# demorest/dspsr

Measured on AMD Instinct MI355X. Metric: Msamples/s dedispersed+folded, higher is better.
Workload: dtype f32

## Files before the change

dspsr_amd/csrc/fb_common.h:

```cpp
#pragma once
#include <math.h>
#include <stdlib.h>

#include <vector>

#include "engine_internal.h"
#include "fold_internal.h"
#include "stamps.h"

namespace dspsr_amd {

struct FbGeom {
  int logM, logR, logT1, logT2, logT3;
  int logX3;
  int four_pass;
  int xblocked;
  uint32_t xblock;
  uint32_t kblock;
  uint64_t xstride;
  int logMf, logMa, logMb, logTm, logTt;
  int real_input, npol;
  uint32_t nsub;
  int logFb2, logFa2;
  uint32_t C, nfilt_pos, nkeep;
  const float2* tw_lo;
  const float2* tw_lo_m;
};

struct FbIn {
  int kind;
  const void* base;
  uint64_t pol_stride;
  uint64_t part_step;
  uint32_t nchan, ichan;
  float scale;
  uint32_t batch;
  uint64_t chan_stride_c;
};

struct FbOut {
  int kind;
  float* base;
  uint64_t chan_stride, pol_stride, part_step;
  int state;
  uint32_t ndim, chan0;
  uint32_t nbin;
  uint64_t prof_span4;
  uint32_t prof_planes;
  uint64_t plane_stride;
  float* part;
  uint32_t nchan_prof;
  uint32_t nseg;
  dspsr_amd_fold* fold;
  const uint32_t* pstart;
  uint32_t nparts_plan;
  uint32_t plan_cap;
  const Interval* piv;
  const uint32_t* blk_first;
  const uint32_t* bin_start;
  uint32_t ts_sf;
  uint32_t ts_magic;
  uint32_t ts_phase0;
  uint32_t ts_G;
  float* ts_carry;
};

struct TsPart { uint32_t phi, ng, rlast, ofirst; };
DEV TsPart ts_part(const FbOut& out, const uint32_t part_in_call, const uint32_t nkeep)
{
  const uint32_t s = out.ts_phase0 + part_in_call * nkeep;
  TsPart p;
  p.ofirst = s / out.ts_sf;
  p.phi = s - p.ofirst * out.ts_sf;
  const uint32_t e = p.phi + nkeep;
  p.ng = (e + out.ts_sf - 1) / out.ts_sf;
  p.rlast = e - (p.ng - 1) * out.ts_sf;
  return p;
}
DEV float sqld(const cf a) { return __fadd_rn(__fmul_rn(a.x, a.x), __fmul_rn(a.y, a.y)); }
DEV void ts_stage(float* __restrict__ stg, const FbOut& out, const TsPart& tp, const uint32_t slo, const uint32_t t, const cf a, const cf b)
{
  const uint32_t tr = t + tp.phi, gq = out.ts_sf == 1 ? tr : __umulhi(tr, out.ts_magic), r = tr - gq * out.ts_sf;
  const float pp = sqld(a), qq = sqld(b);
  if (out.state == DSPSR_AMD_PPQQ) {
    const uint32_t base = ((2 * slo) * out.ts_sf + r) * out.ts_G + gq;
    stg[base] = pp;
    stg[base + out.ts_sf * out.ts_G] = qq;
  } else {
    stg[(slo * out.ts_sf + r) * out.ts_G + gq] = __fadd_rn(pp, qq);
  }
}
// ... 314 lines not shown
  for (int q = 0; q < (NP ? NP : 1); q++) j[1 + q] = (d0 << q) & Lm;
  twiddles_big(t, j, logL, tw, tw_lo);
#pragma unroll
  for (int q = 0; q < 1 + (NP ? NP : 1); q++) t[q].y = -t[q].y;
  if constexpr (R > 1) {
    const cf w1 = t[1];
    const cf w2 = NP >= 2 ? t[1 + (NP >= 2 ? 1 : 0)] : w1, w4 = NP >= 3 ? t[1 + (NP >= 3 ? 2 : 0)] : w1,
             w8 = NP >= 4 ? t[1 + (NP >= 4 ? 3 : 0)] : w1;
    apply_powers<R>(v, w1, w2, w4, w8);
  }
#pragma unroll
  for (int k = 0; k < R; k++) v[k] = cmuls(v[k], t[0]);
}

DEV void detect4(const cf p, const cf q, const int state, float (&r)[4])
{
  const float pp = p.x * p.x + p.y * p.y;
  const float qq = q.x * q.x + q.y * q.y;
  const float re = p.x * q.x + p.y * q.y;
  const float im = p.x * q.y - p.y * q.x;
  if (state == DSPSR_AMD_STOKES) { r[0] = pp + qq; r[1] = pp - qq; r[2] = 2.0f * re; r[3] = 2.0f * im; }
  else { r[0] = pp; r[1] = qq; r[2] = re; r[3] = im; }
}

typedef void (*k1_t)(FbGeom, FbIn, cf*, const cf*, uint64_t, uint32_t, uint32_t, uint32_t);
typedef void (*k2_t)(FbGeom, const cf*, cf*, const cf*, uint32_t, uint32_t, uint32_t);
typedef void (*k3_t)(FbGeom, const cf*, const cf*, FbOut, const cf*, uint64_t, uint32_t, uint32_t);
typedef void (*k3a_t)(FbGeom, const cf*, const cf*, cf*, const cf*, uint32_t, uint32_t);
typedef void (*k3b_t)(FbGeom, const cf*, FbOut, const cf*, uint64_t, uint32_t, uint32_t);

template <int... I> struct iseq {};
template <int N, int... I> struct mkseq : mkseq<N - 1, N - 1, I...> {};
template <int... I> struct mkseq<0, I...> { typedef iseq<I...> type; };

constexpr int full_logt(int logf) { return 14 - logf >= 1 ? 14 - logf : -1; }
constexpr int MAX_LOGF = 13;
typedef mkseq<MAX_LOGF + 1>::type seq_t;
k1_t fb_pick1(int logf, int raww, bool full);
k1_t fb_pick1_dual(int raww);
k2_t fb_pick2(int logf, bool full);
k3_t fb_pick3(int logf, bool full);
k3_t fb_pick3f(int logf, bool full);
k3_t fb_pick3s(int logf, bool full);
k3a_t fb_pick3a(int logf, bool blocked, bool real, bool full);
k3b_t fb_pick3b(int logf, bool foldb, bool full);
typedef void (*k1c_t)(FbGeom, FbIn, cf*, const cf*, uint32_t, uint32_t, uint32_t);
k1c_t fb_pick_col1();
k3_t fb_pick_rinv(int logm, int epi);
void fb_launch_raw_cols(dim3 grid, hipStream_t stream, const FbGeom& g, const FbIn& in, uint16_t* Rt, uint64_t part0);
void fb_launch_sub_split(hipStream_t stream, const SubSplit& p, uint8_t* out, uint32_t ncu);
cf* fb_launch_sub_combine(hipStream_t stream, const FbGeom& g, cf* X, uint32_t nseqs, uint32_t ncu, cf* Xalt, cf* Xout = nullptr, uint32_t mo = 0,
                          uint32_t rm = 1);
void fb_launch_time_combine(hipStream_t stream, const TimeCombine& p, const FbOut& out, uint32_t R, uint32_t ncu);
void fb_launch_raw_transpose(dim3 grid, hipStream_t stream, const FbGeom& g, const FbIn& in, uint16_t* Rt, uint64_t part0);
void fb_launch_float_transpose(dim3 grid, hipStream_t stream, const FbGeom& g, const FbIn& in, cf* Rt, uint64_t part0);
int fb_conv1_check(int logM, size_t* lds_bytes);
int fb_conv1_launch(dspsr_amd_ctx* ctx, int logM, const float* in, uint64_t chan_stride, uint64_t pol_stride, uint64_t in_step,
                    const cf* kern, const FbOut& out, uint32_t nchan, uint32_t nfilt_pos, uint32_t nkeep, uint64_t npart);
constexpr int CONV3_MIN_LOGM = 14, CONV3_MAX_LOGM = 21;
int fb_conv3_check(int logM);
void fb_conv3_response_order(int logM, const cf* natural, cf* ordered);
int fb_conv3_launch(dspsr_amd_ctx* ctx, int logM, const float* in, uint64_t chan_stride, uint64_t pol_stride, uint64_t in_step,
                    const cf* kern, const FbOut& out, uint32_t nchan, uint32_t nfilt_pos, uint32_t nkeep, uint64_t part0, uint32_t nparts,
                    cf* S1, cf* S2);
int fb_plain_check(dspsr_amd_ctx* ctx, int logC, bool real_input, uint32_t npol, size_t* lds_bytes);
int fb_plain_launch(dspsr_amd_ctx* ctx, int logC, bool real_input, uint32_t npol, uint32_t input_nchan, const cf* kern,
                    const FbIn& in, const FbOut& out, uint64_t in_chan_stride, uint64_t npart);

}
```

dspsr_amd/csrc/fb_fwd_cols.hip:

```cpp
#include "fb_common.h"

namespace dspsr_amd {

__global__ __launch_bounds__(256) void k_raw_transpose(const FbGeom g, const FbIn in, uint16_t* __restrict__ Rt,
                                                       const uint64_t part0)
{
  constexpr uint32_t ROWS = 64, COLS = 256, PITCH = COLS / 2 + 1;
  __shared__ uint32_t sm[ROWS * PITCH];
  const uint32_t tid = threadIdx.x;
  const uint32_t M = 1u << g.logM, Rr = 1u << g.logR;
  const int logT = g.logT1;
  const uint32_t nb0 = blockIdx.x * COLS, na0 = blockIdx.y * ROWS;
  const uint32_t nsq = g.real_input ? 1u : g.npol;
  const uint64_t part = blockIdx.z / nsq;
  const uint32_t seq = blockIdx.z % nsq;
  const uint64_t t0 = (part0 + part) * in.part_step;
  const uint32_t ncol = Rr - nb0 < COLS ? Rr - nb0 : COLS, nrow = M - na0 < ROWS ? M - na0 : ROWS;
  if (ncol % 8 == 0) {
    for (uint32_t q = tid; q < nrow * (ncol / 8); q += 256) {
      const uint32_t r = q / (ncol / 8), c8 = (q % (ncol / 8)) * 8;
      const uint64_t t = t0 + (((uint64_t)(na0 + r)) << g.logR) + nb0 + c8;
      uint32_t w[4];
      if (!g.real_input) {
        const uint4* p = (const uint4*)((const uint8_t*)in.base + 4 * t);
        const uint4 s0 = p[0], s1 = p[1];
        const int sh = 16 * seq;
        w[0] = ((s0.x >> sh) & 0xffffu) | (((s0.y >> sh) & 0xffffu) << 16);
        w[1] = ((s0.z >> sh) & 0xffffu) | (((s0.w >> sh) & 0xffffu) << 16);
        w[2] = ((s1.x >> sh) & 0xffffu) | (((s1.y >> sh) & 0xffffu) << 16);
        w[3] = ((s1.z >> sh) & 0xffffu) | (((s1.w >> sh) & 0xffffu) << 16);
      } else if (in.kind == 2) {
        const uint32_t* p = (const uint32_t*)((const uint8_t*)in.base + (t >> 2) * 8);
#pragma unroll
        for (int h = 0; h < 2; h++) {
          const uint32_t p0 = p[2 * h], p1 = p[2 * h + 1];
          w[2 * h] = (p0 & 0xff) | ((p1 & 0xff) << 8) | ((p0 & 0xff00) << 8) | ((p1 & 0xff00) << 16);
          w[2 * h + 1] = ((p0 >> 16) & 0xff) | (((p1 >> 16) & 0xff) << 8) | ((p0 >> 24) << 16) | ((p1 >> 24) << 24);
        }
      } else {
        const uint32_t* p = (const uint32_t*)((const uint8_t*)in.base + 2 * t);
        w[0] = p[0]; w[1] = p[1]; w[2] = p[2]; w[3] = p[3];
      }
#pragma unroll
      for (int h = 0; h < 4; h++) sm[r * PITCH + c8 / 2 + h] = w[h];
    }
  } else {
    for (uint32_t q = tid; q < nrow * (ncol / 2); q += 256) {
      const uint32_t r = q / (ncol / 2), c2 = (q % (ncol / 2)) * 2;
      const uint64_t t = t0 + (((uint64_t)(na0 + r)) << g.logR) + nb0 + c2;
      uint32_t w;
      if (!g.real_input) {
        const uint32_t* p = (const uint32_t*)((const uint8_t*)in.base + 4 * t);
        w = ((p[0] >> (16 * seq)) & 0xffffu) | (((p[1] >> (16 * seq)) & 0xffffu) << 16);
      } else if (in.kind == 2) {
        const uint8_t* b = (const uint8_t*)in.base + (t >> 2) * 8 + (t & 3);
        w = (uint32_t)b[0] | ((uint32_t)b[4] << 8) | ((uint32_t)b[1] << 16) | ((uint32_t)b[5] << 24);
      } else {
        w = *(const uint32_t*)((const uint8_t*)in.base + 2 * t);
      }
      sm[r * PITCH + c2 / 2] = w;
    }
  }
  __syncthreads();
  uint32_t* __restrict__ dst = (uint32_t*)(Rt + (part * nsq + seq) * ((uint64_t)M << g.logR));
  const int logW = logT - 1;
  const uint32_t ntl = ncol >> logT, W = 1u << logW;
  if (logW == 1 && (nrow & 1) == 0) {
    const uint32_t nr2 = nrow >> 1;
    for (uint32_t q = tid; q < ntl * nr2; q += 256) {
      const uint32_t r = (q % nr2) * 2, tl = q / nr2;
      const uint32_t* s0 = &sm[r * PITCH + 2 * tl];
      const uint32_t* s1 = s0 + PITCH;
      *(uint4*)&dst[((((uint64_t)((nb0 >> logT) + tl) << g.logM) + na0 + r) << 1)] = make_uint4(s0[0], s0[1], s1[0], s1[1]);
    }
    return;
  }
  if (logW >= 2) {
    const int logV = logW - 2;
    for (uint32_t q = tid; q < (ntl * nrow) << logV; q += 256) {
      const uint32_t v4 = q & ((1u << logV) - 1), r = (q >> logV) % nrow, tl = (q >> logV) / nrow;
      const uint32_t* s0 = &sm[r * PITCH + (tl << logW) + 4 * v4];
      *(uint4*)&dst[((((uint64_t)((nb0 >> logT) + tl) << g.logM) + na0 + r) << logW) + 4 * v4] = make_uint4(s0[0], s0[1], s0[2], s0[3]);
    }
    return;
  }
  for (uint32_t q = tid; q < ntl * nrow * W; q += 256) {
    const uint32_t wd = q & (W - 1), r = (q >> logW) % nrow, tl = (q >> logW) / nrow;
    dst[((((uint64_t)((nb0 >> logT) + tl) << g.logM) + na0 + r) << logW) + wd] = sm[r * PITCH + (tl << logW) + wd];
  }
}

__global__ __launch_bounds__(256) void k_float_transpose(const FbGeom g, const FbIn in, cf* __restrict__ Rt, const uint64_t part0)
{
  constexpr uint32_t ROWS = FB_FT_ROWS, COLS = FB_FT_COLS, PITCH = COLS + 1;
  __shared__ cf sm[ROWS * PITCH];
  const uint32_t tid = threadIdx.x;
  const uint32_t M = 1u << g.logM, Rr = 1u << g.logR;
  const int logT = g.logT1;
  const uint32_t nb0 = blockIdx.x * COLS, na0 = blockIdx.y * ROWS;
  const uint32_t nsq = g.real_input ? 1u : g.npol;
  const uint64_t part = blockIdx.z / nsq;
  const uint32_t seq = blockIdx.z % nsq;
  const uint64_t t0 = (part0 + part) * in.part_step;
  const uint32_t ncol = Rr - nb0 < COLS ? Rr - nb0 : COLS, nrow = M - na0 < ROWS ? M - na0 : ROWS;
  const float* __restrict__ x = (const float*)in.base;
  if (g.real_input) {
    for (uint32_t q = tid; q < nrow * (ncol / 4); q += 256) {
      const uint32_t r = q / (ncol / 4), c4 = (q % (ncol / 4)) * 4;
      const uint64_t t = t0 + (((uint64_t)(na0 + r)) << g.logR) + nb0 + c4;
      const float4 p0 = ld_stream((const float4*)(x + t)), p1 = ld_stream((const float4*)(x + in.pol_stride + t));
      cf* d = &sm[r * PITCH + c4];
      d[0] = make_float2(p0.x, p1.x); d[1] = make_float2(p0.y, p1.y); d[2] = make_float2(p0.z, p1.z); d[3] = make_float2(p0.w, p1.w);
    }
  } else {
    for (uint32_t q = tid; q < nrow * (ncol / 2); q += 256) {
      const uint32_t r = q / (ncol / 2), c2 = (q % (ncol / 2)) * 2;
      const uint64_t t = t0 + (((uint64_t)(na0 + r)) << g.logR) + nb0 + c2;
      const float4 v = ld_stream((const float4*)(x + seq * in.pol_stride + 2 * t));
      cf* d = &sm[r * PITCH + c2];
      d[0] = make_float2(v.x, v.y); d[1] = make_float2(v.z, v.w);
    }
  }
  __syncthreads();
  cf* __restrict__ dst = Rt + (part * nsq + seq) * ((uint64_t)M << g.logR);
  const uint32_t ntl = ncol >> logT, T = 1u << logT;
  for (uint32_t q = tid; q < ntl * nrow * (T / 2); q += 256) {
    const uint32_t h = q % (T / 2), r = (q / (T / 2)) % nrow, tl = q / ((T / 2) * nrow);
    const cf* s0 = &sm[r * PITCH + (tl << logT) + 2 * h];
    st_stream((float4*)&dst[((((uint64_t)((nb0 >> logT) + tl) << g.logM) + na0 + r) << logT) + 2 * h],
              make_float4(s0[0].x, s0[0].y, s0[1].x, s0[1].y));
  }
}

template <int LOGF, int RAWW, int LOGT>
__global__ __launch_bounds__(512) void k_fwd_cols(const FbGeom g, const FbIn in, cf* __restrict__ A,
                                                  const cf* __restrict__ tw, const uint64_t part0,
                                                  const uint32_t nparts, const uint32_t nseq, const uint32_t run)
{
  typedef FftPlan<LOGF> P;
  extern __shared__ __attribute__((aligned(16))) cf lds[];
  uint32_t tid = threadIdx.x;
  const int logT = LOGT >= 0 ? LOGT : g.logT1, logT2 = g.logT2;
  const uint32_t T = 1u << logT, T2 = 1u << logT2;
  const int logL = LOGF + g.logR;
  const uint64_t L = 1ull << logL;
  const uint32_t ntile = 1u << (g.logR - logT);
  const uint32_t total = ntile * nseq * nparts;
  const int logNt = g.logR - logT;
  auto seq_of = [&](const uint32_t rest) { return nseq == 2 ? (rest & 1u) : 0u; };
  auto part_of = [&](const uint32_t rest) { return nseq == 2 ? (rest >> 1) : rest; };

  auto fetch = [&](const uint32_t item, RawW<RAWW> (&raw)[PTS / 2]) {
    const uint32_t tile = item & (ntile - 1);
    const uint32_t rest = item >> logNt;
    uint32_t seq = seq_of(rest);
    const bool pret = in.kind == 3 || in.kind == 5;
    uint64_t t0 = pret ? ((uint64_t)rest * ntile + tile) * ((uint64_t)T << LOGF)
                       : (part0 + part_of(rest)) * in.part_step + tile * T;
    if constexpr (RAWW == 4) {
      if (in.batch) {
        const uint32_t c = rest % in.batch, ps = rest / in.batch;
        seq = ps % (uint32_t)g.npol;
        t0 = (part0 + ps / (uint32_t)g.npol) * in.part_step + c * in.chan_stride_c + tile * T;
      }
    }
    constexpr uint32_t MS = 1u << (LOGF - P::LOGR1);
    const uint64_t step = pret ? ((uint64_t)MS << logT) : ((uint64_t)MS << g.logR);
#pragma unroll
    for (int g2 = 0; g2 < P::G1; g2 += 2) {
      const uint32_t eb = P::G1 * tid + g2;
      const uint64_t tb = t0 + (eb & (T - 1)) + (pret ? (uint64_t)((eb >> logT) << logT) : (((uint64_t)(eb >> logT)) << g.logR));
#pragma unroll
      for (int i = 0; i < P::R1; i++) raw[(g2 / 2) * P::R1 + i] = fetch_pair<RAWW>(g, in, seq, tb + i * step);
    }
  };

  const uint32_t ltw_off = lds_pad(PTS * blockDim.x) + 8;
  ltw_fill<LOGF>(lds, ltw_off, tw, threadIdx.x, blockDim.x);
  const uint32_t co_swz = (PTS * blockDim.x) >= 256 ? 1u : 0u;
  const uint32_t co_l0 = 2 * threadIdx.x;
  const uint32_t co_n2 = LOGT >= 0 ? (2u << (LOGF + LOGT - LOG_PTS)) : 2 * blockDim.x;
  const int co_sh = logT + logT2;
  const bool co_fast = (co_n2 & 63) == 0 && (co_n2 >> co_sh) != 0 && (co_n2 & ((1u << co_sh) - 1)) == 0;
  const uint32_t co_lds = lds_pad(co_l0 ^ (((co_l0 >> 4) & co_swz) << 3)), co_lstep = co_n2 + ((co_n2 >> 6) << 2);
  const uint32_t co_goff = (uint32_t)(((((uint64_t)(co_l0 >> co_sh) << g.logR) << logT2) + (co_l0 & ((1u << co_sh) - 1))) * sizeof(cf));
  const uint64_t co_gstep = ((uint64_t)(co_n2 >> co_sh) << g.logR) << logT2;
  auto copy_out = [&](const uint32_t tile, cf* __restrict__ Aseq) {
    const uint32_t swz = co_swz;
    const uint32_t nthr = blockDim.x;
    if (co_fast) {
      const char* __restrict__ gb = (const char*)(Aseq + ((uint64_t)(tile * T) << logT2));
#pragma unroll
      for (int j4 = 0; j4 < PTS / 2; j4 += 4) {
        float4 pr[4];
#pragma unroll
        for (int q = 0; q < 4; q++) pr[q] = *(const float4*)&lds[co_lds + (j4 + q) * co_lstep];
        __builtin_amdgcn_sched_barrier(0);
#pragma unroll
        for (int q = 0; q < 4; q++) st_stream((float4*)(gb + (uint64_t)(j4 + q) * co_gstep * sizeof(cf) + co_goff), pr[q]);
        __builtin_amdgcn_sched_barrier(0);
      }
    } else {
#pragma unroll 4
      for (int jj = 0; jj < PTS / 2; jj++) {
        const uint32_t l = 2 * (tid + jj * nthr);
        const uint32_t blkA = l >> (logT + logT2), within = l & ((1u << (logT + logT2)) - 1);
        const float4 pr = *(const float4*)&lds[lds_pad(l ^ (((l >> 4) & swz) << 3))];
        st_stream((float4*)&Aseq[((((uint64_t)blkA << g.logR) + tile * T) << logT2) + within], pr);
      }
    }
// ... 37 lines not shown
          float* __restrict__ d1 = (float*)&lds[b1 + k * sp];
          d0[0] = v[k].x[0]; d0[1] = v[k].y[0];
          d1[0] = v[k].x[1]; d1[1] = v[k].y[1];
        }
      } else {
#pragma unroll
        for (int k = 0; k < R; k++) {
          const uint32_t ka = k * pstride + p;
          const uint32_t l = ((((ka >> logT2) << logT) + col) << logT2) | (ka & (T2 - 1));
          lds[img(l)] = cx2_lo(v[k]);
          lds[img(l + T2)] = cx2_hi(v[k]);
        }
      }
    };
    wgfft<LOGF, -1, true>(lds, ltw_off, tid, logT, x, store);
    __syncthreads();
    FB_ST(1, 3);
    copy_out(tile, Aseq);
    FB_ST(1, 4);
    FB_ST_TILE(1, 5);
    if (!more) break;
    item = next;
  }
  FB_ST_END(1);
}

struct KeepOut {
  cx2* o;
  uint32_t p0;
  int h;
  template <int R> DEV void operator()(const uint32_t, const uint32_t p, const uint32_t, cx2 (&v)[R])
  {
    static_assert(R == 2, "k_fwd_cols_dual: radix-2 last stage");
    if (h == 0) p0 = p;
    o[2 * h] = v[0];
    o[2 * h + 1] = v[1];
  }
};
template <int RAWW>
__global__ __launch_bounds__(512) void k_fwd_cols_dual(const FbGeom g, const FbIn in, cf* __restrict__ A,
                                                       const cf* __restrict__ tw, const uint64_t part0,
                                                       const uint32_t nparts, const uint32_t nseq, const uint32_t run)
{
  constexpr int LOGF = 13, LOGT = 1;
  typedef FftPlan<LOGF> P;
  static_assert(P::REM == 1 && PTS / 2 / 2 == 8, "k_fwd_cols_dual: 2^13-point columns, radix-2 last stage");
  extern __shared__ __attribute__((aligned(16))) cf lds[];
  uint32_t tid = threadIdx.x;
  const int logT2 = g.logT2;
  const uint32_t T = 2, T2 = 1u << logT2;
  const int logL = LOGF + g.logR;
  const uint64_t L = 1ull << logL;
  const int logNp = g.logR - LOGT - 1;
  const uint32_t npair = 1u << logNp, ntile = npair << 1;
  const uint32_t total = npair * nseq * nparts;
  auto seq_of = [&](const uint32_t rest) { return nseq == 2 ? (rest & 1u) : 0u; };
  auto part_of = [&](const uint32_t rest) { return nseq == 2 ? (rest >> 1) : rest; };
  auto fetch = [&](const uint32_t item, const uint32_t sub, RawW<RAWW> (&raw)[PTS / 2]) {
    const uint32_t tile = ((item & (npair - 1)) << 1) | sub;
    const uint32_t rest = item >> logNp;
    const uint32_t seq = seq_of(rest);
    const bool pret = in.kind == 3 || in.kind == 5;
    const uint64_t t0 = pret ? ((uint64_t)rest * ntile + tile) * ((uint64_t)T << LOGF) : (part0 + part_of(rest)) * in.part_step + tile * T;
    constexpr uint32_t MS = 1u << (LOGF - P::LOGR1);
    const uint64_t step = pret ? ((uint64_t)MS << LOGT) : ((uint64_t)MS << g.logR);
#pragma unroll
    for (int g2 = 0; g2 < P::G1; g2 += 2) {
      const uint32_t eb = P::G1 * tid + g2;
      const uint64_t tb = t0 + (eb & (T - 1)) + (pret ? (uint64_t)((eb >> LOGT) << LOGT) : (((uint64_t)(eb >> LOGT)) << g.logR));
#pragma unroll
      for (int i = 0; i < P::R1; i++) raw[(g2 / 2) * P::R1 + i] = fetch_pair<RAWW>(g, in, seq, tb + i * step);
    }
  };
  const uint32_t ltw_off = lds_pad(PTS * blockDim.x) + 8;
  ltw_fill<LOGF>(lds, ltw_off, tw, threadIdx.x, blockDim.x);
  auto img = [](const uint32_t l) { return l + ((l >> 5) << 1); };
  const int sh = 2 + logT2;
  const uint32_t co_l0 = 2 * threadIdx.x;
  const uint32_t co_lds = img(co_l0), co_lstep = img(1024);
  const uint64_t co_goff = (((uint64_t)(co_l0 >> sh) << g.logR) << logT2) + (co_l0 & ((1u << sh) - 1));
  const uint64_t co_gstep = ((uint64_t)(1024u >> sh) << g.logR) << logT2;
  uint32_t item, next;
  uint32_t j = 0;
  if (!persistent_item(blockIdx.x, gridDim.x, j, run, total, item)) return;
  RawW<RAWW> raw0[PTS / 2], raw1[PTS / 2];
  fetch(item, 0, raw0);
  fetch(item, 1, raw1);
  for (;;) {
    asm volatile("" : "+v"(tid));
    const bool more = persistent_item(blockIdx.x, gridDim.x, ++j, run, total, next);
    const uint32_t seq_cur = seq_of(item >> logNp);
    cx2 o0[PTS / 2], o1[PTS / 2];
    uint32_t p0;
    {
      cx2 x[NPAIR];
#pragma unroll
      for (int h = 0; h < NPAIR; h++) {
        cf a, b;
        decode_pair<RAWW>(g, in, raw0[h], a, b, seq_cur);
        x[h] = make_cx2(a, b);
      }
      if (more) fetch(next, 0, raw0);
      KeepOut keep{o0, 0u, 0};
      wgfft<LOGF, -1, false>(lds, ltw_off, tid, LOGT, x, keep);
      p0 = keep.p0;
    }
    {
      cx2 x[NPAIR];
#pragma unroll
      for (int h = 0; h < NPAIR; h++) {
        cf a, b;
        decode_pair<RAWW>(g, in, raw1[h], a, b, seq_cur);
        x[h] = make_cx2(a, b);
      }
      if (more) fetch(next, 1, raw1);
      KeepOut keep{o1, 0u, 0};
// ... 150 lines not shown
  const int logLs = g.logM + g.logR;
  const uint32_t Ls = 1u << logLs, L = Ls * R;
  const uint32_t X3m = (1u << g.logX3) - 1, Mm = (1u << g.logM) - 1;
  const uint64_t n = (uint64_t)nseqs << logLs;
  for (uint64_t i = (uint64_t)blockIdx.x * blockDim.x + threadIdx.x; i < n; i += (uint64_t)gridDim.x * blockDim.x) {
    const uint32_t o = (uint32_t)(i & (Ls - 1));
    cf* __restrict__ base = X + (i >> logLs) * (uint64_t)L + o;
    const uint32_t t = o >> g.logX3, m = t & Mm, sp = ((t >> g.logM) << g.logX3) | (o & X3m);
    const uint32_t k = (sp << g.logM) + m;
    cf gq[R];
    gq[0] = base[0];
#pragma unroll
    for (int c = 1; c < R; c++) {
      gq[c] = cmul(base[(uint64_t)c << logLs], twiddle_odd<R>((uint32_t)c * k, logLs, wr));
    }
#pragma unroll
    for (int q = 0; q < R; q++) {
      cf acc = gq[0];
#pragma unroll
      for (int c = 1; c < R; c++) {
        const cf v = cmul(gq[c], wr.w[(c * q) % R]);
        acc.x += v.x; acc.y += v.y;
      }
      if constexpr (!MSUB) {
        base[(uint64_t)q << logLs] = acc;
      } else {
        const uint32_t kk = k + ((uint32_t)q << logLs);
        const uint32_t Rr = (uint32_t)R << g.logR, N = g.real_input ? L >> 1 : L;
        const bool up = kk > N;
        const uint32_t kq = up ? L - kk : kk;
        const uint32_t cc = kq / mo, mm = kq - cc * mo, mi = mm / rm, r = mm - mi * rm, s = cc * rm + r;
        uint32_t row, bin;
        if (kk == N && g.real_input) { row = Rr >> 1; bin = 0; }
        else if (!up) { row = s; bin = mi; }
        else if (mi) { row = Rr - 1 - s; bin = (1u << g.logM) - mi; }
        else { row = Rr - s; bin = 0; }
        Xout[(i >> logLs) * (uint64_t)L + (((((uint64_t)(row >> g.logX3) << g.logM) + bin) << g.logX3) | (row & X3m))] = acc;
      }
    }
  }
}

template <int... I> static k1_t pick1(int logf, int raww, bool full, iseq<I...>)
{
  static const k1_t t4[] = {k_fwd_cols<I, 4, -1>...};
  static const k1_t t1[] = {k_fwd_cols<I, 1, -1>...};
  static const k1_t f4[] = {k_fwd_cols<I, 4, full_logt(I)>...};
  static const k1_t f1[] = {k_fwd_cols<I, 1, full_logt(I)>...};
  return full ? (raww == 1 ? f1[logf] : f4[logf]) : (raww == 1 ? t1[logf] : t4[logf]);
}
k1_t fb_pick1(int logf, int raww, bool full) { return pick1(logf, raww, full, seq_t()); }
k1_t fb_pick1_dual(int raww) { return raww == 1 ? k_fwd_cols_dual<1> : nullptr; }

void fb_launch_raw_transpose(dim3 grid, hipStream_t stream, const FbGeom& g, const FbIn& in, uint16_t* Rt, uint64_t part0)
{
  hipLaunchKernelGGL(k_raw_transpose, grid, dim3(256), 0, stream, g, in, Rt, part0);
}
void fb_launch_float_transpose(dim3 grid, hipStream_t stream, const FbGeom& g, const FbIn& in, cf* Rt, uint64_t part0)
{
  hipLaunchKernelGGL(k_float_transpose, grid, dim3(256), 0, stream, g, in, Rt, part0);
}
template <bool MSUB>
__global__ __launch_bounds__(256) void k_sub_combine_any(const FbGeom g, const cf* __restrict__ X, const uint32_t nseqs,
                                                         cf* __restrict__ Xout, const uint32_t mo, const uint32_t rm, const OddTw wr)
{
  const int logLs = g.logM + g.logR;
  const uint32_t R = wr.R, Ls = 1u << logLs, L = Ls * R;
  const uint32_t X3m = (1u << g.logX3) - 1, Mm = (1u << g.logM) - 1;
  const uint64_t n = (uint64_t)nseqs * L;
  for (uint64_t i = (uint64_t)blockIdx.x * blockDim.x + threadIdx.x; i < n; i += (uint64_t)gridDim.x * blockDim.x) {
    const uint32_t o = (uint32_t)(i & (Ls - 1));
    const uint64_t rest = i >> logLs;
    const uint32_t q = (uint32_t)(rest % R);
    const uint64_t seq = rest / R;
    const cf* __restrict__ base = X + seq * (uint64_t)L + o;
    const uint32_t t = o >> g.logX3, m = t & Mm, sp = ((t >> g.logM) << g.logX3) | (o & X3m);
    const uint32_t k = (sp << g.logM) + m, kk = k + (q << logLs);
    cf acc = base[0];
    for (uint32_t c = 1; c < R; c++) {
      const cf v = cmul(base[(uint64_t)c << logLs], twiddle_odd_rt((uint64_t)c * kk, logLs, wr));
      acc.x += v.x; acc.y += v.y;
    }
    if constexpr (!MSUB) {
      Xout[seq * (uint64_t)L + ((uint64_t)q << logLs) + o] = acc;
    } else {
      const uint32_t Rr = R << g.logR, N = g.real_input ? L >> 1 : L;
      const bool up = kk > N;
      const uint32_t kq = up ? L - kk : kk;
      const uint32_t cc = kq / mo, mm = kq - cc * mo, mi = mm / rm, r = mm - mi * rm, s = cc * rm + r;
      uint32_t row, bin;
      if (kk == N && g.real_input) { row = Rr >> 1; bin = 0; }
      else if (!up) { row = s; bin = mi; }
      else if (mi) { row = Rr - 1 - s; bin = (1u << g.logM) - mi; }
      else { row = Rr - s; bin = 0; }
      Xout[seq * (uint64_t)L + (((((uint64_t)(row >> g.logX3) << g.logM) + bin) << g.logX3) | (row & X3m))] = acc;
    }
  }
}

template <int KIND, int EB>
static void sub_split_launch(hipStream_t stream, const SubSplit& p, uint8_t* out, uint32_t ncu)
{
  constexpr uint32_t N = 16 / EB;
  const bool fast = (p.sub_stride % 16) == 0 && ((p.nper * EB) % 16) == 0 && ((p.wlen * EB) % 16) == 0 && ((uintptr_t)out % 16) == 0;
  uint64_t m_lo = 0;
  if (fast && p.wlen >= N) {
    m_lo = (p.wlen / N) * N;
    switch (p.R) {
      case 3: hipLaunchKernelGGL((k_sub_split<KIND, EB, 3>), dim3(8 * ncu), dim3(256), 0, stream, p, out); break;
// ... 36 lines not shown
```

dspsr_amd/csrc/filterbank.hip:

```cpp
#include "fb_common.h"
#include <initializer_list>

namespace dspsr_amd {

constexpr int LOG_POINTS_DEFAULT = 14;

static inline int ilog2(uint64_t v) { int l = 0; while ((1ull << l) < v) l++; return l; }
static inline bool ispow2(uint64_t v) { return v && !(v & (v - 1)); }

struct dspsr_amd_filterbank_impl {
  dspsr_amd_ctx* ctx;
  dspsr_amd_filterbank_config cfg;
  FbGeom g;
  uint64_t N, L;
  uint32_t nseq, max_parts;
  uint32_t nt1, nt2, nt3, nt4 = 0, ncu, wg3 = 1, wg1 = 1;
  size_t lds1, lds2, lds3, lds4 = 0;
  uint64_t part_elems = 0;
  cf* A = nullptr;
  cf* X = nullptr;
  cf* kernel = nullptr;
  cf* tw_lo = nullptr;
  cf* tw_lo_m = nullptr;
  uint16_t* Rt = nullptr;
// ... 674 lines not shown

template <typename F>
static int fb_each_group(dspsr_amd_filterbank* fb, const FbIn& in, const FbOut& out, uint64_t npart, uint64_t chan_stride, F&& group)
{
  const FbGeom& g = fb->g;
  for (uint32_t ichan = 0; ichan < fb->cfg.input_nchan; ichan++) {
    FbIn ci = in;
    if (in.kind == 0) ci.base = (const float*)in.base + ichan * chan_stride;
    ci.ichan = ichan;
    ci.nchan = fb->cfg.input_nchan;
    FbOut co = out;
    co.chan0 = ichan * g.C;
    const cf* kern = fb->kernel ? fb->kernel + (uint64_t)ichan * fb->N : nullptr;
    uint32_t nb = 0;
    for (uint64_t part0 = 0; part0 < npart; part0 += nb) {
      nb = fb_group_parts(npart - part0, fb->max_parts, g, fb->nseq, g);
      const int rc = group(ci, co, kern, part0, nb);
      if (rc != DSPSR_AMD_OK) return rc;
    }
  }
  return fb_launch_status(fb->ctx);
}

static int fb_subband_group(dspsr_amd_filterbank* fb, const FbIn& in, uint32_t ichan, uint64_t chan_stride, const FbOut& co,
                            const cf* kern, k3_t k3, uint64_t part0, uint32_t nb, uint32_t rp, bool fused_segmented)
{
  dspsr_amd_ctx* ctx = fb->ctx;
  const FbGeom& g = fb->g;
  const uint32_t R = g.nsub, ndim = g.real_input ? 1u : 2u, Rr = 1u << g.logR, M = 1u << g.logM;
  const uint64_t step = in.part_step * rp;
  const uint64_t wlen = rp > 1 ? fb->L / R : ((uint64_t)(nb - 1) * step + fb->L) / R, nper = rp > 1 ? (uint64_t)nb * wlen : wlen;
  const size_t es = in.kind == 0 ? (size_t)g.npol * ndim * sizeof(float) : (size_t)g.npol * ndim;
  const size_t sub_stride = (nper * es + 15) & ~(size_t)15;
  if (!grow_device_buffer(ctx->stream, fb->dsub, fb->dsub_bytes, sub_stride * R))
    return fb_fail(ctx, DSPSR_AMD_ENOMEM, "dspsr_amd_filterbank_perform: hipMalloc of %zu sub-sequence bytes failed", sub_stride * R);
  SubSplit sp = {in.kind, in.base, in.kind == 0 ? (uint64_t)ichan * chan_stride : 0, in.pol_stride,
                 fb->cfg.input_nchan, ichan, (uint32_t)g.npol, ndim, part0 * in.part_step, nper, R, sub_stride,
                 rp > 1 ? nb : 1u, wlen, step};
  fb_launch_sub_split(ctx->stream, sp, fb->dsub, fb->ncu);
  const uint64_t Ls = fb->L / R;
  for (uint32_t c = 0; c < R; c++) {
    FbIn cs = in;
    cs.kind = in.kind == 0 ? 0 : 1;
    cs.base = fb->dsub + (size_t)c * sub_stride;
    cs.pol_stride = in.kind == 0 ? nper * ndim : 0;
    cs.part_step = rp > 1 ? wlen : step / R;
    cs.nchan = 1; cs.ichan = 0;
    FbPass1 p1;
    const int rc = fb_pass1(fb, cs, 0, false, true, &p1);
    if (rc != DSPSR_AMD_OK) return rc;
    k1_t k1s = p1.raww == 1 ? fb->k1_w1 : fb->k1_w4;
    if (!k1s) return fb_fail(ctx, DSPSR_AMD_EINVAL, "dspsr_amd_filterbank_perform: no kernel for this geometry");
    FbIn cr = cs;
    if (p1.regroup == FB_REGROUP_RAW) {
      fb_launch_raw_transpose(dim3((Rr + 255) / 256, (M + 63) / 64, nb * fb->nseq), ctx->stream, g, cs, fb->Rt, 0);
      cr.kind = 3; cr.base = fb->Rt;
    } else if (p1.regroup == FB_REGROUP_FLOAT) {
      cf* ft = fb->A + (size_t)nb * fb->nseq * Ls;
      fb_launch_float_transpose(dim3((Rr + FB_FT_COLS - 1) / FB_FT_COLS, (M + FB_FT_ROWS - 1) / FB_FT_ROWS, nb * fb->nseq), ctx->stream, g, cs, ft, 0);
      cr.kind = 5; cr.base = ft;
    }
    const uint64_t n1s = (uint64_t)(Rr >> g.logT1) * fb->nseq * nb, n2s = (uint64_t)(M >> g.logT2) * fb->nseq * nb;
    hipLaunchKernelGGL(k1s, dim3(grid_for(n1s, fb->ncu * fb->wg1)), dim3(fb->nt1), fb->lds1, ctx->stream, g, cr, fb->A, ctx->tw, 0ull,
                       nb, fb->nseq, 32u);
    hipLaunchKernelGGL(fb->k2, dim3(grid_for(n2s, fb->ncu)), dim3(fb->nt2), fb->lds2, ctx->stream, g, fb->A, fb->X + c * Ls,
                       ctx->tw, nb, fb->nseq, 4u);
  }
  const uint64_t n3s = (uint64_t)(g.C >> g.logT3) * nb;
  if (fb->msub) {
    const uint64_t Mi = 1ull << g.logM, xe = (uint64_t)fb->max_parts * fb->nseq * fb->L,
                   ye = (uint64_t)g.C * g.npol * fb->max_parts * Mi;
    if (!fb->Xp && hipMalloc((void**)&fb->Xp, xe * sizeof(cf)) != hipSuccess)
      return fb_fail(ctx, DSPSR_AMD_ENOMEM, "dspsr_amd_filterbank_perform: hipMalloc of the pseudo-channel spectrum failed");
    if (!fb->Y && hipMalloc((void**)&fb->Y, ye * sizeof(cf)) != hipSuccess)
      return fb_fail(ctx, DSPSR_AMD_ENOMEM, "dspsr_amd_filterbank_perform: hipMalloc of the pseudo-channel time series failed");
    (void)fb_launch_sub_combine(ctx->stream, g, fb->X, nb * fb->nseq, fb->ncu, nullptr, fb->Xp, fb->out_M, fb->msub);
    FbOut yo = {1, (float*)fb->Y, (uint64_t)g.npol * fb->max_parts * Mi * 2, (uint64_t)fb->max_parts * Mi * 2, Mi * 2, 0, 2, 0};
    hipLaunchKernelGGL(fb->k3, dim3(grid_for(n3s, fb->ncu * fb->wg3)), dim3(fb->nt3), fb->lds3, ctx->stream, g, fb->Xp, kern, yo, ctx->tw,
                       0ull, nb, nb);
    TimeCombine tc = {fb->Y, (uint64_t)g.npol * fb->max_parts * Mi, (uint64_t)fb->max_parts * Mi, (uint32_t)g.logM, fb->out_M,
                      fb->out_nfilt_pos, fb->out_nkeep, fb->out_C, (uint32_t)g.npol, part0, nb, rp, make_odd_tw(fb->msub)};
    FbOut cu = co;
    cu.chan0 = ichan * fb->out_C;
    if (cu.kind == 1 || cu.kind == 2) fb_launch_time_combine(ctx->stream, tc, cu, fb->msub, fb->ncu);
    return DSPSR_AMD_OK;
  }
  if (rp != 1) return fb_fail(ctx, DSPSR_AMD_EINVAL, "dspsr_amd_filterbank_perform: part step %llu is not a multiple of %u",
                              (unsigned long long)in.part_step, R);
  const cf* Xc = fb_launch_sub_combine(ctx->stream, g, fb->X, nb * fb->nseq, fb->ncu, fb->A);
  if (co.kind == 3) return fb_launch_fused(fb, k3, Xc, kern, co, part0, nb, fused_segmented);
  hipLaunchKernelGGL(k3, dim3(grid_for(co.kind == 5 ? n3s / nb : n3s, fb->ncu * fb->wg3)), dim3(fb->nt3), fb->lds3, ctx->stream, g, Xc,
                     kern, co, ctx->tw, part0, nb, nb);
  return DSPSR_AMD_OK;
}

static int fb_run_subbands(dspsr_amd_filterbank* fb, const FbIn& in, const FbOut& out, uint64_t npart, uint64_t chan_stride, k3_t k3)
{
  const uint32_t R = fb->g.nsub;
  if (in.kind == 4)
    return fb_fail(fb->ctx, DSPSR_AMD_EINVAL, "dspsr_amd_filterbank_perform: 16-bit UWB blocks need power-of-two nchan_subband and "
                   "freq_res (k_sub_split de-interleaves 8-bit and float32 input)");
  auto gcd = [](uint32_t x, uint32_t y) { while (y) { const uint32_t t = x % y; x = y; y = t; } return x; };
  const uint32_t rp = (in.part_step % R) ? R / gcd((uint32_t)(in.part_step % R), R) : 1u;
  const bool fused_segmented = out.kind == 3 && dspsr_amd_filterbank_fold_is_fused(fb) == 2;
  return fb_each_group(fb, in, out, npart, chan_stride, [&](const FbIn& ci, const FbOut& co, const cf* kern, uint64_t part0, uint32_t nb) {
    for (uint32_t q = 0; q < rp && q < nb; q++) {
      const int rc = fb_subband_group(fb, in, ci.ichan, chan_stride, co, kern, k3, part0 + q, (nb - q + rp - 1) / rp, rp, fused_segmented);
      if (rc != DSPSR_AMD_OK) return rc;
    }
    return DSPSR_AMD_OK;
  });
}

static int fb_run_two_pass(dspsr_amd_filterbank* fb, const FbIn& in, const FbOut& out, uint64_t npart, uint64_t chan_stride)
{
  dspsr_amd_ctx* ctx = fb->ctx;
  const FbGeom& g = fb->g;
  const uint32_t Fb = 1u << g.logFb2, tiles = g.C >> g.logFb2;
  const bool fused_segmented = out.kind == 3 && dspsr_amd_filterbank_fold_is_fused(fb) == 2;
  return fb_each_group(fb, in, out, npart, chan_stride, [&](const FbIn& ci, const FbOut& co, const cf* kern, uint64_t part0, uint32_t nb) {
    FbIn cr = ci;
    cr.kind = 3;
    cr.base = fb->Rt;
    if (fb->k1c) {
      fb_launch_raw_cols(dim3((uint32_t)(fb->L / 8192), nb), ctx->stream, g, ci, fb->Rt, part0);
      const uint64_t n1c = (uint64_t)Fb * 2 * nb;
      hipLaunchKernelGGL(fb->k1c, dim3(grid_for(n1c, fb->ncu)), dim3(512), fb->lds1c, ctx->stream, g, cr, fb->A, ctx->tw, nb, 2u, 32u);
    } else {
      const FbGeom& q = fb->g1t;
      const uint32_t Fa = 1u << q.logM;
      fb_launch_raw_transpose(dim3((Fb + 255) / 256, (Fa + 63) / 64, nb * 2), ctx->stream, q, ci, fb->Rt, part0);
      const uint64_t n1t = (uint64_t)(Fb >> q.logT1) * 2 * nb;
      hipLaunchKernelGGL(fb->k1t, dim3(grid_for(n1t, fb->ncu)), dim3(fb->nt1t), fb->lds1t, ctx->stream, q, cr, fb->A, ctx->tw, part0,
                         nb, 2u, 32u);
    }
    if (co.kind == 3) return fb_launch_fused(fb, fb->k2rf, fb->A, kern, co, part0, nb, fused_segmented, true);
    if (co.kind == 5)
      hipLaunchKernelGGL(fb->k2rs, dim3(grid_for(tiles, fb->ncu)), dim3(512), fb->lds2r, ctx->stream, g, fb->A, kern, co, ctx->tw, part0,
                         nb, nb);
    else
      hipLaunchKernelGGL(fb->k2r, dim3(grid_for((uint64_t)tiles * nb, fb->ncu)), dim3(512), fb->lds2r, ctx->stream, g, fb->A, kern, co,
                         ctx->tw, part0, nb, nb);
    return DSPSR_AMD_OK;
  });
}

static int fb_run_tiles(dspsr_amd_filterbank* fb, const FbIn& in, const FbOut& out, uint64_t npart, uint64_t chan_stride,
                        const FbPass1& p1, const FbPassKernels& k)
{
  dspsr_amd_ctx* ctx = fb->ctx;
  const FbGeom& g = fb->g;
  const uint32_t Rr = 1u << g.logR, M = 1u << g.logM;
  const bool fused_segmented = out.kind == 3 && dspsr_amd_filterbank_fold_is_fused(fb) == 2;
  return fb_each_group(fb, in, out, npart, chan_stride, [&](const FbIn& ci, const FbOut& co, const cf* kern, uint64_t part0, uint32_t nb) {
    const uint64_t n1 = (uint64_t)(Rr >> g.logT1) * fb->nseq * nb, n2 = (uint64_t)(M >> g.logT2) * fb->nseq * nb,
                   n3 = g.four_pass ? 0 : (uint64_t)(g.C >> g.logT3) * nb;
    const uint32_t run1 = 32, run2 = 4, run3 = nb;
    FbIn c1 = ci;
    if (p1.regroup == FB_REGROUP_RAW) {
      fb_launch_raw_transpose(dim3((Rr + 255) / 256, (M + 63) / 64, nb * fb->nseq), ctx->stream, g, ci, fb->Rt, part0);
      c1.kind = 3; c1.base = fb->Rt;
    } else if (p1.regroup == FB_REGROUP_FLOAT) {
      fb_launch_float_transpose(dim3((Rr + FB_FT_COLS - 1) / FB_FT_COLS, (M + FB_FT_ROWS - 1) / FB_FT_ROWS, nb * fb->nseq), ctx->stream, g, ci, fb->X, part0);
      c1.kind = 5; c1.base = fb->X;
    }
    if (k.k1d)
      hipLaunchKernelGGL(k.k1d, dim3(grid_for(n1 / 2, fb->ncu * fb->wg1)), dim3(fb->nt1), fb->lds1, ctx->stream, g, c1, fb->A, ctx->tw,
                         part0, nb, fb->nseq, run1 / 2 ? run1 / 2 : 1u);
    else
      hipLaunchKernelGGL(k.k1, dim3(grid_for(n1, fb->ncu * fb->wg1)), dim3(fb->nt1), fb->lds1, ctx->stream, g, c1, fb->A, ctx->tw,
                         part0, nb, fb->nseq, run1);
    uint64_t p23auto = (512ull << 20) / (fb->part_elems * sizeof(cf));
    if (p23auto < 1) p23auto = 1;
    const uint32_t p23sub = (g.four_pass || (co.kind == 3 && fused_segmented)) ? nb : (uint32_t)(p23auto < nb ? p23auto : nb);
    if (p23sub < nb) {
      for (uint32_t s0 = 0; s0 < nb; s0 += p23sub) {
        const uint32_t ns = nb - s0 < p23sub ? nb - s0 : p23sub;
        const uint64_t off = (uint64_t)s0 * fb->part_elems;
        const uint64_t n2s = (uint64_t)(M >> g.logT2) * fb->nseq * ns;
        const uint64_t n3s = co.kind == 5 ? (uint64_t)(g.C >> g.logT3) : (uint64_t)(g.C >> g.logT3) * ns;
        hipLaunchKernelGGL(fb->k2, dim3(grid_for(n2s, fb->ncu)), dim3(fb->nt2), fb->lds2, ctx->stream, g, fb->A + off,
                           fb->X + off, ctx->tw, ns, fb->nseq, run2);
        if (co.kind == 3) {
          const int rc = fb_launch_fused(fb, k.k3, fb->X + off, kern, co, part0 + s0, ns, fused_segmented);
          if (rc != DSPSR_AMD_OK) return rc;
        } else {
          hipLaunchKernelGGL(k.k3, dim3(grid_for(n3s, fb->ncu * fb->wg3)), dim3(fb->nt3), fb->lds3, ctx->stream, g, fb->X + off, kern, co,
                             ctx->tw, part0 + s0, ns, ns);
        }
      }
      return DSPSR_AMD_OK;
    }
    hipLaunchKernelGGL(fb->k2, dim3(grid_for(n2, fb->ncu)), dim3(fb->nt2), fb->lds2, ctx->stream, g, fb->A, fb->X,
                       ctx->tw, nb, fb->nseq, run2);
    if (!g.four_pass) {
      if (co.kind == 3) return fb_launch_fused(fb, k.k3, fb->X, kern, co, part0, nb, fused_segmented);
      const uint64_t items3 = co.kind == 5 ? (uint64_t)(g.C >> g.logT3) : n3;
      hipLaunchKernelGGL(k.k3, dim3(grid_for(items3, fb->ncu * fb->wg3)), dim3(fb->nt3), fb->lds3, ctx->stream, g, fb->X, kern, co,
                         ctx->tw, part0, nb, run3);
      return DSPSR_AMD_OK;
    }
    const uint64_t n3a = ((uint64_t)g.C << (g.logMb - g.logTm)) * nb, n3b = ((uint64_t)g.C << (g.logMa - g.logTt)) * nb;
    hipLaunchKernelGGL(fb->k3a, dim3(grid_for(n3a, fb->ncu)), dim3(fb->nt3), fb->lds3, ctx->stream, g, fb->X, kern,
                       fb->A, ctx->tw, nb, 8u);
    if (co.kind == 4) {
      const int rc = fb_plan_ready(fb, co.fold);
      if (rc != DSPSR_AMD_OK) return rc;
    }
    hipLaunchKernelGGL(k.k3b, dim3(grid_for(n3b, fb->ncu)), dim3(fb->nt4), fb->lds4, ctx->stream, g, fb->A, co,
                       ctx->tw, part0, nb, 8u);
    if (co.kind == 4 && part0 + nb == npart)
      return fold_segment_combine(co.fold, fb->msum, co.chan0, g.C, (uint32_t)npart, g.nkeep, g.nfilt_pos, g.logTt, g.logMa,
                                  g.logMb, co.bin_start, co.piv);
    return DSPSR_AMD_OK;
  });
}

// ... 311 lines not shown
```

Measured before the change: 96590.

## Share raw-transpose buffer across overlapping parts instead of per-part copies

Adds an Rt layout abstraction with explicit tile, seq and part strides. When consecutive parts overlap (part_step is a multiple of the row length), the raw transpose writes one shared padded row range for all parts instead of duplicating the overlapping rows per part. The first-pass kernels then read through the layout strides. This is meant to cut redundant transpose traffic and Rt memory, at the cost of extra stride arithmetic and a more complex layout contract with the first-pass kernels.

```diff
diff --git a/dspsr_amd/csrc/fb_common.h b/dspsr_amd/csrc/fb_common.h
--- a/dspsr_amd/csrc/fb_common.h
+++ b/dspsr_amd/csrc/fb_common.h
@@ -5,6 +5,7 @@
 #include <vector>
 
 #include "engine_internal.h"
+#include "fb_rt_layout.h"
 #include "fold_internal.h"
 #include "stamps.h"
 
@@ -36,7 +37,16 @@
   float scale;
   uint32_t batch;
   uint64_t chan_stride_c;
-};
+  uint64_t rt_tile_stride = 0, rt_seq_stride = 0, rt_part_stride = 0;
+};
+static inline void fb_set_rt(FbIn& in, int kind, const void* base, const RtLayout& l)
+{
+  in.kind = kind;
+  in.base = base;
+  in.rt_tile_stride = l.tile_stride;
+  in.rt_seq_stride = l.seq_stride;
+  in.rt_part_stride = l.part_stride;
+}
 
 struct FbOut {
   int kind;
@@ -457,7 +467,8 @@
 cf* fb_launch_sub_combine(hipStream_t stream, const FbGeom& g, cf* X, uint32_t nseqs, uint32_t ncu, cf* Xalt, cf* Xout = nullptr, uint32_t mo = 0,
                           uint32_t rm = 1);
 void fb_launch_time_combine(hipStream_t stream, const TimeCombine& p, const FbOut& out, uint32_t R, uint32_t ncu);
-void fb_launch_raw_transpose(dim3 grid, hipStream_t stream, const FbGeom& g, const FbIn& in, uint16_t* Rt, uint64_t part0);
+void fb_launch_raw_transpose(hipStream_t stream, const FbGeom& g, const FbIn& in, uint16_t* Rt, uint64_t part0, uint32_t nb, uint32_t nseq,
+                             const RtLayout& lay);
 void fb_launch_float_transpose(dim3 grid, hipStream_t stream, const FbGeom& g, const FbIn& in, cf* Rt, uint64_t part0);
 int fb_conv1_check(int logM, size_t* lds_bytes);
 int fb_conv1_launch(dspsr_amd_ctx* ctx, int logM, const float* in, uint64_t chan_stride, uint64_t pol_stride, uint64_t in_step,
diff --git a/dspsr_amd/csrc/fb_fwd_cols.hip b/dspsr_amd/csrc/fb_fwd_cols.hip
--- a/dspsr_amd/csrc/fb_fwd_cols.hip
+++ b/dspsr_amd/csrc/fb_fwd_cols.hip
@@ -3,19 +3,21 @@
 namespace dspsr_amd {
 
 __global__ __launch_bounds__(256) void k_raw_transpose(const FbGeom g, const FbIn in, uint16_t* __restrict__ Rt,
-                                                       const uint64_t part0)
+                                                       const uint64_t part0, const RtLayout lay)
 {
   constexpr uint32_t ROWS = 64, COLS = 256, PITCH = COLS / 2 + 1;
   __shared__ uint32_t sm[ROWS * PITCH];
   const uint32_t tid = threadIdx.x;
-  const uint32_t M = 1u << g.logM, Rr = 1u << g.logR;
+  static_assert(ROWS == RT_ROW_BLOCK, "k_raw_transpose: the layout pads the rows of a tile to whole blocks");
+  const uint32_t Rr = 1u << g.logR;
   const int logT = g.logT1;
   const uint32_t nb0 = blockIdx.x * COLS, na0 = blockIdx.y * ROWS;
   const uint32_t nsq = g.real_input ? 1u : g.npol;
   const uint64_t part = blockIdx.z / nsq;
   const uint32_t seq = blockIdx.z % nsq;
   const uint64_t t0 = (part0 + part) * in.part_step;
-  const uint32_t ncol = Rr - nb0 < COLS ? Rr - nb0 : COLS, nrow = M - na0 < ROWS ? M - na0 : ROWS;
+  const uint32_t ncol = Rr - nb0 < COLS ? Rr - nb0 : COLS, nrow = lay.rows - na0 < ROWS ? lay.rows - na0 : ROWS;
+  const uint32_t rpad = lay.rows_padded;
   if (ncol % 8 == 0) {
     for (uint32_t q = tid; q < nrow * (ncol / 8); q += 256) {
       const uint32_t r = q / (ncol / 8), c8 = (q % (ncol / 8)) * 8;
@@ -62,7 +64,7 @@
     }
   }
   __syncthreads();
-  uint32_t* __restrict__ dst = (uint32_t*)(Rt + (part * nsq + seq) * ((uint64_t)M << g.logR));
+  uint32_t* __restrict__ dst = (uint32_t*)(Rt + part * lay.part_stride + seq * lay.seq_stride);
   const int logW = logT - 1;
   const uint32_t ntl = ncol >> logT, W = 1u << logW;
   if (logW == 1 && (nrow & 1) == 0) {
@@ -71,7 +73,7 @@
       const uint32_t r = (q % nr2) * 2, tl = q / nr2;
       const uint32_t* s0 = &sm[r * PITCH + 2 * tl];
       const uint32_t* s1 = s0 + PITCH;
-      *(uint4*)&dst[((((uint64_t)((nb0 >> logT) + tl) << g.logM) + na0 + r) << 1)] = make_uint4(s0[0], s0[1], s1[0], s1[1]);
+      *(uint4*)&dst[(((uint64_t)((nb0 >> logT) + tl) * rpad + na0 + r) << 1)] = make_uint4(s0[0], s0[1], s1[0], s1[1]);
     }
     return;
   }
@@ -80,13 +82,13 @@
     for (uint32_t q = tid; q < (ntl * nrow) << logV; q += 256) {
       const uint32_t v4 = q & ((1u << logV) - 1), r = (q >> logV) % nrow, tl = (q >> logV) / nrow;
       const uint32_t* s0 = &sm[r * PITCH + (tl << logW) + 4 * v4];
-      *(uint4*)&dst[((((uint64_t)((nb0 >> logT) + tl) << g.logM) + na0 + r) << logW) + 4 * v4] = make_uint4(s0[0], s0[1], s0[2], s0[3]);
+      *(uint4*)&dst[(((uint64_t)((nb0 >> logT) + tl) * rpad + na0 + r) << logW) + 4 * v4] = make_uint4(s0[0], s0[1], s0[2], s0[3]);
     }
     return;
   }
   for (uint32_t q = tid; q < ntl * nrow * W; q += 256) {
     const uint32_t wd = q & (W - 1), r = (q >> logW) % nrow, tl = (q >> logW) / nrow;
-    dst[((((uint64_t)((nb0 >> logT) + tl) << g.logM) + na0 + r) << logW) + wd] = sm[r * PITCH + (tl << logW) + wd];
+    dst[(((uint64_t)((nb0 >> logT) + tl) * rpad + na0 + r) << logW) + wd] = sm[r * PITCH + (tl << logW) + wd];
   }
 }
 
@@ -155,7 +157,7 @@
     const uint32_t rest = item >> logNt;
     uint32_t seq = seq_of(rest);
     const bool pret = in.kind == 3 || in.kind == 5;
-    uint64_t t0 = pret ? ((uint64_t)rest * ntile + tile) * ((uint64_t)T << LOGF)
+    uint64_t t0 = pret ? part_of(rest) * in.rt_part_stride + seq * in.rt_seq_stride + tile * in.rt_tile_stride
                        : (part0 + part_of(rest)) * in.part_step + tile * T;
     if constexpr (RAWW == 4) {
       if (in.batch) {
@@ -299,7 +301,7 @@
   const int logL = LOGF + g.logR;
   const uint64_t L = 1ull << logL;
   const int logNp = g.logR - LOGT - 1;
-  const uint32_t npair = 1u << logNp, ntile = npair << 1;
+  const uint32_t npair = 1u << logNp;
   const uint32_t total = npair * nseq * nparts;
   auto seq_of = [&](const uint32_t rest) { return nseq == 2 ? (rest & 1u) : 0u; };
   auto part_of = [&](const uint32_t rest) { return nseq == 2 ? (rest >> 1) : rest; };
@@ -308,7 +310,8 @@
     const uint32_t rest = item >> logNp;
     const uint32_t seq = seq_of(rest);
     const bool pret = in.kind == 3 || in.kind == 5;
-    const uint64_t t0 = pret ? ((uint64_t)rest * ntile + tile) * ((uint64_t)T << LOGF) : (part0 + part_of(rest)) * in.part_step + tile * T;
+    const uint64_t t0 = pret ? part_of(rest) * in.rt_part_stride + seq * in.rt_seq_stride + tile * in.rt_tile_stride
+                             : (part0 + part_of(rest)) * in.part_step + tile * T;
     constexpr uint32_t MS = 1u << (LOGF - P::LOGR1);
     const uint64_t step = pret ? ((uint64_t)MS << LOGT) : ((uint64_t)MS << g.logR);
 #pragma unroll
@@ -565,9 +568,11 @@
 k1_t fb_pick1(int logf, int raww, bool full) { return pick1(logf, raww, full, seq_t()); }
 k1_t fb_pick1_dual(int raww) { return raww == 1 ? k_fwd_cols_dual<1> : nullptr; }
 
-void fb_launch_raw_transpose(dim3 grid, hipStream_t stream, const FbGeom& g, const FbIn& in, uint16_t* Rt, uint64_t part0)
-{
-  hipLaunchKernelGGL(k_raw_transpose, grid, dim3(256), 0, stream, g, in, Rt, part0);
+void fb_launch_raw_transpose(hipStream_t stream, const FbGeom& g, const FbIn& in, uint16_t* Rt, uint64_t part0, uint32_t nb, uint32_t nseq,
+                             const RtLayout& lay)
+{
+  const dim3 grid(((1u << g.logR) + 255) / 256, (lay.rows + RT_ROW_BLOCK - 1) / RT_ROW_BLOCK, lay.shared ? nseq : nb * nseq);
+  hipLaunchKernelGGL(k_raw_transpose, grid, dim3(256), 0, stream, g, in, Rt, part0, lay);
 }
 void fb_launch_float_transpose(dim3 grid, hipStream_t stream, const FbGeom& g, const FbIn& in, cf* Rt, uint64_t part0)
 {
diff --git a/dspsr_amd/csrc/fb_rt_layout.h b/dspsr_amd/csrc/fb_rt_layout.h
--- /dev/null
+++ b/dspsr_amd/csrc/fb_rt_layout.h
@@ -0,0 +1,66 @@
+#pragma once
+#include <stdint.h>
+
+#if defined(__HIPCC__)
+#define RT_HD __host__ __device__ inline
+#else
+#define RT_HD inline
+#endif
+
+namespace dspsr_amd {
+
+constexpr uint32_t RT_ROW_BLOCK = 64;
+
+struct RtLayout {
+  uint32_t shared;
+  uint32_t logT1;
+  uint32_t rows;
+  uint32_t rows_padded;
+  uint64_t tile_stride, seq_stride, part_stride;
+};
+
+RT_HD RtLayout rt_layout_per_part(const int logM, const int logR, const int logT1, const uint32_t nseq)
+{
+  RtLayout l;
+  l.shared = 0;
+  l.logT1 = (uint32_t)logT1;
+  l.rows = l.rows_padded = 1u << logM;
+  l.tile_stride = (uint64_t)l.rows << logT1;
+  l.seq_stride = (uint64_t)l.rows << logR;
+  l.part_stride = l.seq_stride * nseq;
+  return l;
+}
+
+RT_HD RtLayout rt_layout_shared(const int logM, const int logR, const int logT1, const uint32_t nb, const uint64_t rstep)
+{
+  RtLayout l;
+  l.shared = 1;
+  l.logT1 = (uint32_t)logT1;
+  l.rows = (uint32_t)(rstep * (nb - 1)) + (1u << logM);
+  l.rows_padded = (l.rows + RT_ROW_BLOCK - 1) & ~(RT_ROW_BLOCK - 1);
+  l.tile_stride = (uint64_t)l.rows_padded << logT1;
+  l.seq_stride = (uint64_t)l.rows_padded << logR;
+  l.part_stride = rstep << logT1;
+  return l;
+}
+
+RT_HD uint64_t rt_elems(const RtLayout& l, const int logR, const uint32_t nseq, const uint32_t nb)
+{
+  return l.shared ? l.seq_stride * nseq : ((uint64_t)l.rows << logR) * nseq * nb;
+}
+
+RT_HD bool rt_takes_shared(const int logM, const int logR, const uint32_t nb, const uint64_t part_step, const uint32_t y_max = 65535)
+{
+  if (nb < 2 || (part_step & ((1ull << logR) - 1)) != 0) return false;
+  const uint64_t rstep = part_step >> logR, M = 1ull << logM;
+  if (rstep == 0 || rstep > M) return false;
+  const uint64_t rows = rstep * (nb - 1) + M, padded = (rows + RT_ROW_BLOCK - 1) & ~(uint64_t)(RT_ROW_BLOCK - 1);
+  return padded <= M * nb && padded / RT_ROW_BLOCK <= y_max;
+}
+
+RT_HD uint64_t rt_offset(const RtLayout& l, const uint32_t part, const uint32_t seq, const uint32_t tile, const uint32_t na, const uint32_t col)
+{
+  return part * l.part_stride + seq * l.seq_stride + tile * l.tile_stride + ((uint64_t)na << l.logT1) + col;
+}
+
+}
diff --git a/dspsr_amd/csrc/filterbank.hip b/dspsr_amd/csrc/filterbank.hip
--- a/dspsr_amd/csrc/filterbank.hip
+++ b/dspsr_amd/csrc/filterbank.hip
@@ -750,13 +750,14 @@
     k1_t k1s = p1.raww == 1 ? fb->k1_w1 : fb->k1_w4;
     if (!k1s) return fb_fail(ctx, DSPSR_AMD_EINVAL, "dspsr_amd_filterbank_perform: no kernel for this geometry");
     FbIn cr = cs;
+    const RtLayout lay = rt_layout_per_part(g.logM, g.logR, g.logT1, fb->nseq);
     if (p1.regroup == FB_REGROUP_RAW) {
-      fb_launch_raw_transpose(dim3((Rr + 255) / 256, (M + 63) / 64, nb * fb->nseq), ctx->stream, g, cs, fb->Rt, 0);
-      cr.kind = 3; cr.base = fb->Rt;
+      fb_launch_raw_transpose(ctx->stream, g, cs, fb->Rt, 0, nb, fb->nseq, lay);
+      fb_set_rt(cr, 3, fb->Rt, lay);
     } else if (p1.regroup == FB_REGROUP_FLOAT) {
       cf* ft = fb->A + (size_t)nb * fb->nseq * Ls;
       fb_launch_float_transpose(dim3((Rr + FB_FT_COLS - 1) / FB_FT_COLS, (M + FB_FT_ROWS - 1) / FB_FT_ROWS, nb * fb->nseq), ctx->stream, g, cs, ft, 0);
-      cr.kind = 5; cr.base = ft;
+      fb_set_rt(cr, 5, ft, lay);
     }
     const uint64_t n1s = (uint64_t)(Rr >> g.logT1) * fb->nseq * nb, n2s = (uint64_t)(M >> g.logT2) * fb->nseq * nb;
     hipLaunchKernelGGL(k1s, dim3(grid_for(n1s, fb->ncu * fb->wg1)), dim3(fb->nt1), fb->lds1, ctx->stream, g, cr, fb->A, ctx->tw, 0ull,
@@ -826,8 +827,9 @@
       hipLaunchKernelGGL(fb->k1c, dim3(grid_for(n1c, fb->ncu)), dim3(512), fb->lds1c, ctx->stream, g, cr, fb->A, ctx->tw, nb, 2u, 32u);
     } else {
       const FbGeom& q = fb->g1t;
-      const uint32_t Fa = 1u << q.logM;
-      fb_launch_raw_transpose(dim3((Fb + 255) / 256, (Fa + 63) / 64, nb * 2), ctx->stream, q, ci, fb->Rt, part0);
+      const RtLayout lay = rt_layout_per_part(q.logM, q.logR, q.logT1, 2);
+      fb_launch_raw_transpose(ctx->stream, q, ci, fb->Rt, part0, nb, 2, lay);
+      fb_set_rt(cr, 3, fb->Rt, lay);
       const uint64_t n1t = (uint64_t)(Fb >> q.logT1) * 2 * nb;
       hipLaunchKernelGGL(fb->k1t, dim3(grid_for(n1t, fb->ncu)), dim3(fb->nt1t), fb->lds1t, ctx->stream, q, cr, fb->A, ctx->tw, part0,
                          nb, 2u, 32u);
@@ -855,12 +857,14 @@
                    n3 = g.four_pass ? 0 : (uint64_t)(g.C >> g.logT3) * nb;
     const uint32_t run1 = 32, run2 = 4, run3 = nb;
     FbIn c1 = ci;
+    RtLayout lay = rt_layout_per_part(g.logM, g.logR, g.logT1, fb->nseq);
     if (p1.regroup == FB_REGROUP_RAW) {
-      fb_launch_raw_transpose(dim3((Rr + 255) / 256, (M + 63) / 64, nb * fb->nseq), ctx->stream, g, ci, fb->Rt, part0);
-      c1.kind = 3; c1.base = fb->Rt;
+      if (rt_takes_shared(g.logM, g.logR, nb, ci.part_step)) lay = rt_layout_shared(g.logM, g.logR, g.logT1, nb, ci.part_step >> g.logR);
+      fb_launch_raw_transpose(ctx->stream, g, ci, fb->Rt, part0, nb, fb->nseq, lay);
+      fb_set_rt(c1, 3, fb->Rt, lay);
     } else if (p1.regroup == FB_REGROUP_FLOAT) {
       fb_launch_float_transpose(dim3((Rr + FB_FT_COLS - 1) / FB_FT_COLS, (M + FB_FT_ROWS - 1) / FB_FT_ROWS, nb * fb->nseq), ctx->stream, g, ci, fb->X, part0);
-      c1.kind = 5; c1.base = fb->X;
+      fb_set_rt(c1, 5, fb->X, lay);
     }
     if (k.k1d)
       hipLaunchKernelGGL(k.k1d, dim3(grid_for(n1 / 2, fb->ncu * fb->wg1)), dim3(fb->nt1), fb->lds1, ctx->stream, g, c1, fb->A, ctx->tw,
```

After: 98440 (median of 6 runs). +1.9%, better.
